# HiKapok/DAN

Hardware: AMD Instinct MI355X
Metric: 640x640 images/sec/node (train fwd+bwd) (higher is better)
Workload: dtype bf16; 1 GPU; S3FD VGG-16 backbone + 6 detection heads, 640x640 bf16 training (fwd+bwd+SGD), batch 16 per GPU; global_batch=16, parallelism=dp1, anchors_per_image=34125, step_launch=eager, rccl_ranks=1, weight_gradient_stream=True

## Files before the change

### dan_amd/_lib.py

```python
import ctypes
import os

import torch

_HERE = os.path.dirname(os.path.abspath(__file__))
ACT_NAME = os.environ.get("DANHIP_DTYPE", "bf16").lower()
if ACT_NAME not in ("bf16", "fp16"):
    raise ValueError("DANHIP_DTYPE must be bf16 or fp16, got %r" % ACT_NAME)
ACT_DTYPE = torch.float16 if ACT_NAME == "fp16" else torch.bfloat16
SO_PATH = os.path.join(_HERE, "libdanhip_f16.so" if ACT_NAME == "fp16" else "libdanhip.so")
if os.environ.get("DANHIP_LIB_PATH"):
    SO_PATH = os.path.abspath(os.environ["DANHIP_LIB_PATH"])

F32, BF16 = 0, 1
SPLIT3 = 3


class ConvDesc(ctypes.Structure):
    _fields_ = [(n, ctypes.c_int32) for n in ("N", "H", "W", "Cin", "Ho", "Wo", "Cout", "kh", "kw", "stride")]


class ConvPitch(ctypes.Structure):
    _fields_ = [(n, ctypes.c_int32) for n in ("x_pitch", "y_pitch", "aux_pitch")]

# ... 26 lines not shown
    "danhip_maxpool2x2_split3": [P, P, I32, I32, I32, I32, P],
    "danhip_l2norm_split3": [P, P, P, I64, I32, I32, I32, P],
    "danhip_conv3x3_c3_f32_split3": [P, P, P, P, I32, I32, I32, I32, ctypes.c_int, I32, P],
    "danhip_conv2d_fwd_split": [DESC, P, P, P, P, ctypes.c_int, ctypes.c_int, I32, P, ctypes.c_size_t, P],
    "danhip_l2norm_fwd_f32": [P, P, P, I64, I32, P],
    "danhip_resize_bilinear_add_fwd_f32": [P, P, P, I32, I32, I32, I32, I32, I32, P],
    "danhip_avgpool2x2s1_same_fwd_f32": [P, P, I32, I32, I32, I32, P],
    "danhip_deform_sample_fwd_f32": [P, P, P, I32, I32, I32, I32, I32, I32, I32, I32, I32, P],
    "danhip_conv2d_bwd_data": [DESC, P, P, P, P, ctypes.c_int, P],
    "danhip_conv2d_bwd_data_ws": [DESC, P, P, P, P, ctypes.c_int, P, ctypes.c_size_t, P],
    "danhip_conv2d_bwd_data_bits": [DESC, P, P, P, P, ctypes.c_int, P],
    "danhip_conv2d_bwd_data_bits_first": [DESC, P, P, P, P, I32, P, P, P],
    "danhip_relu_bits": [P, P, I64, I32, P],
    "danhip_conv2d_fwd_relu_bits": [DESC, P, P, P, P, P, P, P, P],
    "danhip_conv2d_bwd_weight": [DESC, P, P, P, P, I32, P],
    "danhip_conv2d_bwd_weight_ws": [DESC, P, P, P, P, I32, P, ctypes.c_size_t, P],
    "danhip_avgpool2x2s1_same_fwd_strided": [P, I32, P, I32, I32, I32, I32, I32, ctypes.c_int, P],
    "danhip_avgpool2x2s1_same_bwd_strided": [P, I32, P, I32, I32, I32, I32, I32, P],
    "danhip_add16": [P, P, P, I64, P],
    "danhip_residual_bwd": [P, P, P, P, P, ctypes.c_int, I64, P],
    "danhip_conv2d_fwd_strided": [DESC, P, P, P, P, ctypes.c_int, I32, ctypes.POINTER(ConvPitch), P, ctypes.c_size_t, P],
    "danhip_conv2d_bwd_data_strided": [DESC, P, P, P, P, ctypes.c_int, ctypes.POINTER(ConvPitch), P, ctypes.c_size_t, P],
    "danhip_conv2d_fwd_concat2": [DESC, P, P, I32, I32, P, P, P, ctypes.c_int, P],
    "danhip_conv2d_bwd_weight_strided": [DESC, P, P, P, P, I32, ctypes.POINTER(ConvPitch), P, ctypes.c_size_t, P],
    "danhip_relu_bwd_bias_grad": [P, P, P, I64, I32, P],
    "danhip_maxpool2x2_fwd": [P, P, I32, I32, I32, I32, P],
    "danhip_maxpool2x2_fwd_arg": [P, P, P, I32, I32, I32, I32, P],
    "danhip_maxpool2x2_bwd_arg": [P, P, P, I32, I32, I32, I32, ctypes.c_int, P],
    "danhip_conv2d_fwd_pool_arg": [DESC, P, P, P, P, P, P, P],
    "danhip_conv2d_fwd_relu_bits_arg": [DESC, P, P, P, P, P, P, P, P, P],
    "danhip_maxpool2x2_bwd": [P, P, P, I32, I32, I32, I32, ctypes.c_int, P],
    "danhip_l2norm_fwd": [P, P, P, I64, I32, P],
    "danhip_l2norm_bwd": [P, P, P, P, P, I64, I32, ctypes.c_int, ctypes.c_int, P],
    "danhip_preprocess_u8": [P, P, I64, P],
    "danhip_resize_bilinear_add_fwd": [P, P, P, I32, I32, I32, I32, I32, I32, P],
    "danhip_resize_bilinear_add_bwd": [P, P, I32, I32, I32, I32, I32, I32, ctypes.c_int, P],
    "danhip_avgpool2x2s1_same_fwd": [P, P, I32, I32, I32, I32, P],
    "danhip_avgpool2x2s1_same_bwd": [P, P, P, I32, I32, I32, I32, ctypes.c_int, P],
    "danhip_slice_deliver": [P, I32, I32, I32, P, I32, P, I32, ctypes.c_int, I64, P],
    "danhip_batchnorm_fwd_train": [P, P, P, P, P, P, P, P, I64, I32, FL, FL, ctypes.c_int, P, P],
    "danhip_batchnorm_fwd_infer": [P, P, P, P, P, P, I64, I32, ctypes.c_int, P],
    "danhip_batchnorm_bwd": [P, P, P, P, P, P, P, P, I64, I32, P],
    "danhip_dynamic_anchor_routing_eval": [P, P, P, P, I64, I32, I32, I32, I32, I32, P, P, P, ctypes.c_size_t, P],
    "danhip_dynamic_anchor_routing_train": [P, P, P, P, I64, I32, I32, I32, I32, I32, FL, FL, ctypes.c_uint64, ctypes.c_uint64, P, P, P, P,
                                            ctypes.c_size_t, P],
    "danhip_nms": [P, I32, I32, I32, FL, P, P, P],
    "danhip_argsort_desc_f32": [P, I64, I32, P, P, ctypes.c_size_t, P],
    "danhip_augment_preprocess": [P, I32, I32, I32, ctypes.POINTER(ctypes.c_int32), ctypes.POINTER(ctypes.c_float), I32, I32, I32, I32, I32, P, I32, I32,
                                  P, ctypes.c_size_t, P],
    "danhip_deform_psroi_pool_fwd": [P, P, P, P, P, I32, I32, I32, I32, I32, I32, I32, I32, I32, FL, FL, I32, I32, P],
    "danhip_deform_psroi_pool_bwd": [P, P, P, P, P, P, P, I32, I32, I32, I32, I32, I32, I32, I32, I32, I32, FL, FL, I32, I32, P],
    "danhip_maxpool3x3s2_same_fwd": [P, P, I32, I32, I32, I32, P],
    "danhip_maxpool3x3s2_same_bwd": [P, P, P, I32, I32, I32, I32, P],
    "danhip_resize_u8_linear": [P, I32, I32, P, I32, I32, I32, ctypes.c_double, ctypes.c_double, P],
    "danhip_bbox_vote": [P, P, I32, I32, ctypes.c_double, I32, P, P, P, ctypes.c_size_t, P],
    "danhip_deform_sample_fwd": [P, P, P, I32, I32, I32, I32, I32, I32, I32, I32, I32, P],
    "danhip_deform_sample_bwd": [P, P, P, P, P, I32, I32, I32, I32, I32, I32, I32, I32, I32, ctypes.c_int, P, ctypes.c_size_t, P],
    "danhip_deform_conv_fwd": [P, P, P, P, P, I32, I32, I32, I32, I32, I32, I32, I32, I32, I32, ctypes.c_int, P, ctypes.c_size_t, P],
    "danhip_deform_conv_bwd": [P, P, P, P, P, P, P, P, I32, I32, I32, I32, I32, I32, I32, I32, I32, I32, ctypes.c_int, P, ctypes.c_size_t, P],
    "danhip_deform_conv_bwd_with_col": [P, P, P, P, P, P, P, P, P, I32, I32, I32, I32, I32, I32, I32, I32, I32, I32, ctypes.c_int, P, ctypes.c_size_t, P],
    "danhip_deform_conv_bwd_deliver": [P, P, P, P, P, P, P, P, P, I32, I32, I32, I32, I32, I32, I32, I32, I32, I32, ctypes.c_int, ctypes.c_int, P, ctypes.c_size_t, P],
    "danhip_cast_pad_f32_to_bf16": [P, P, P, I64, I32, I32, P],
    "danhip_head_split_fwd": [P, P, P, I32, I32, I32, I32, I32, I32, I32, P],
    "danhip_head_split_bwd": [P, P, P, P, I32, I32, I32, I32, I32, I32, I32, P],
    "danhip_hard_neg_select": [P, P, P, P, P, P, I32, I32, FL, ctypes.c_int, P],
    "danhip_detection_loss_fwd": [P, P, P, P, P, P, P, P, I32, I32, P],
# ... 133 lines not shown
```

### dan_amd/csrc/elementwise.hip

```cpp
#include "common.h"

namespace {

__device__ __forceinline__ float wave_sum(float v) {
#pragma unroll
  for (int o = 32; o > 0; o >>= 1) v += __shfl_xor(v, o, 64);
  return v;
}

struct bf8 { uint4 v; };
__device__ __forceinline__ void unpack8(const uint4& u, float* f) {
  const unsigned w[4] = {u.x, u.y, u.z, u.w};
#pragma unroll
  for (int i = 0; i < 4; ++i) unpack2bf(w[i], f[2 * i], f[2 * i + 1]);
}
__device__ __forceinline__ uint4 pack8(const float* f) {
  uint4 u;
  u.x = pack2bf(f[0], f[1]); u.y = pack2bf(f[2], f[3]); u.z = pack2bf(f[4], f[5]); u.w = pack2bf(f[6], f[7]);
  return u;
}

__global__ void relu_bwd_bias_kernel(bf16_t* __restrict__ dy, const bf16_t* __restrict__ y, float* __restrict__ db, long M, int C) {
  const int cg = C / 8;
  const int tpr = blockDim.x / cg > 0 ? blockDim.x / cg : 1;
// ... 130 lines not shown
  const long nwaves = (long)gridDim.x * (blockDim.x >> 6);
  float gm[VPL][8];
#pragma unroll
  for (int v = 0; v < VPL; ++v)
#pragma unroll
    for (int i = 0; i < 8; ++i) gm[v][i] = gamma[(v * LPP + l) * 8 + i];
  for (long p0 = wave * PPW; p0 < M; p0 += nwaves * PPW) {
    const long pix = p0 + sub;
    const bool ok = pix < M;
    float f[VPL][8];
    float ss = 0.f;
#pragma unroll
    for (int v = 0; v < VPL; ++v) {
      if (ok) unpack8(*reinterpret_cast<const uint4*>(x + pix * C + (v * LPP + l) * 8), f[v]);
      else
#pragma unroll
        for (int i = 0; i < 8; ++i) f[v][i] = 0.f;
#pragma unroll
      for (int i = 0; i < 8; ++i) ss += f[v][i] * f[v][i];
    }
    ss = pixel_sum<LPP, VPL>(ss);
    const float inv = rsqrtf(fmaxf(ss, 1e-10f));
    if (ok) {
#pragma unroll
      for (int v = 0; v < VPL; ++v) {
#pragma unroll
        for (int i = 0; i < 8; ++i) f[v][i] = f[v][i] * inv * gm[v][i];
        *reinterpret_cast<uint4*>(y + pix * C + (v * LPP + l) * 8) = pack8(f[v]);
      }
    }
  }
}

template <int LPP, int VPL>
__global__ void l2norm_bwd_kernel(const bf16_t* __restrict__ x, const float* __restrict__ gamma, const bf16_t* __restrict__ dy,
                                  bf16_t* __restrict__ dx, float* __restrict__ dgamma, long M, int C, int accumulate, int relu_mask) {
  constexpr int PPW = 64 / LPP;
  extern __shared__ float sg[];
  for (int c = threadIdx.x; c < C; c += blockDim.x) sg[c] = 0.f;
  __syncthreads();
  const int lane = threadIdx.x & 63;
  const int sub = lane / LPP, l = lane % LPP;
  const long wave = (long)blockIdx.x * (blockDim.x >> 6) + (threadIdx.x >> 6);
  const long nwaves = (long)gridDim.x * (blockDim.x >> 6);
  float gm[VPL][8], dg[VPL][8];
#pragma unroll
  for (int v = 0; v < VPL; ++v)
#pragma unroll
    for (int i = 0; i < 8; ++i) { gm[v][i] = gamma[(v * LPP + l) * 8 + i]; dg[v][i] = 0.f; }
  for (long p0 = wave * PPW; p0 < M; p0 += nwaves * PPW) {
    const long pix = p0 + sub;
    const bool ok = pix < M;
    float f[VPL][8], g[VPL][8];
    float ss = 0.f, dot = 0.f;
#pragma unroll
    for (int v = 0; v < VPL; ++v) {
      const long o = pix * C + (v * LPP + l) * 8;
      if (ok) {
        unpack8(*reinterpret_cast<const uint4*>(x + o), f[v]);
        unpack8(*reinterpret_cast<const uint4*>(dy + o), g[v]);
      } else {
#pragma unroll
        for (int i = 0; i < 8; ++i) { f[v][i] = 0.f; g[v][i] = 0.f; }
      }
#pragma unroll
      for (int i = 0; i < 8; ++i) { ss += f[v][i] * f[v][i]; dot += g[v][i] * gm[v][i] * f[v][i]; }
    }
    ss = pixel_sum<LPP, VPL>(ss);
    dot = pixel_sum<LPP, VPL>(dot);
    const float inv = rsqrtf(fmaxf(ss, 1e-10f));
    const float k = (ss > 1e-10f) ? dot * inv * inv * inv : 0.f;
    if (ok) {
#pragma unroll
      for (int v = 0; v < VPL; ++v) {
        const long o = pix * C + (v * LPP + l) * 8;
        float r[8], old[8];
        if (accumulate) unpack8(*reinterpret_cast<const uint4*>(dx + o), old);
#pragma unroll
        for (int i = 0; i < 8; ++i) {
          float t = gm[v][i] * inv * g[v][i] - f[v][i] * k;
          if (relu_mask && !(f[v][i] > 0.f)) t = 0.f;
          if (accumulate) t += old[i];
          r[i] = t;
          dg[v][i] += g[v][i] * f[v][i] * inv;
        }
        *reinterpret_cast<uint4*>(dx + o) = pack8(r);
      }
    }
  }
#pragma unroll
  for (int v = 0; v < VPL; ++v)
#pragma unroll
    for (int i = 0; i < 8; ++i) atomicAdd(sg + (v * LPP + l) * 8 + i, dg[v][i]);
  __syncthreads();
  for (int c = threadIdx.x; c < C; c += blockDim.x) atomicAdd(dgamma + c, sg[c]);
}

__global__ void preprocess_kernel(const unsigned char* __restrict__ img, bf16_t* __restrict__ out, long npix) {
  for (long p = (long)blockIdx.x * blockDim.x + threadIdx.x; p < npix; p += (long)gridDim.x * blockDim.x) {
    const float r = (float)img[p * 3] - 123.68f, g = (float)img[p * 3 + 1] - 116.78f, b = (float)img[p * 3 + 2] - 103.94f;
    float f[8] = {b, g, r, 0, 0, 0, 0, 0};
    *reinterpret_cast<uint4*>(out + p * 8) = pack8(f);
  }
}

__global__ void cast_pad_kernel(const float* __restrict__ src, const bf16_t* __restrict__ relu_y, bf16_t* __restrict__ dst, long rows, int c_src,
                                int c_dst) {
  const long total = rows * c_dst;
  for (long i = (long)blockIdx.x * blockDim.x + threadIdx.x; i < total; i += (long)gridDim.x * blockDim.x) {
    const long r = i / c_dst;
    const int c = (int)(i % c_dst);
    float v = c < c_src ? src[r * c_src + c] : 0.f;
    if (relu_y && c < c_src && !(bf2f(relu_y[r * c_src + c]) > 0.f)) v = 0.f;
    dst[i] = f2bf(v);
  }
}

inline int grid_for(long total, int block, int cap = 8192) {
  long b = (total + block - 1) / block;
  if (b > cap) b = cap;
  if (b < 1) b = 1;
  return (int)b;
}

}

// ... 211 lines not shown
  const dim3 g((unsigned)blocks), b(256);
  switch (C) {
    case 64: hipLaunchKernelGGL((l2norm_fwd_kernel<8, 1>), g, b, 0, s, x, gamma, y, (long)M, C); break;
    case 128: hipLaunchKernelGGL((l2norm_fwd_kernel<16, 1>), g, b, 0, s, x, gamma, y, (long)M, C); break;
    case 256: hipLaunchKernelGGL((l2norm_fwd_kernel<32, 1>), g, b, 0, s, x, gamma, y, (long)M, C); break;
    case 512: hipLaunchKernelGGL((l2norm_fwd_kernel<64, 1>), g, b, 0, s, x, gamma, y, (long)M, C); break;
    default: hipLaunchKernelGGL((l2norm_fwd_kernel<64, 2>), g, b, 0, s, x, gamma, y, (long)M, C); break;
  }
  DH_LAUNCH_CHECK();
  return DANHIP_OK;
}

extern "C" int danhip_l2norm_bwd(const uint16_t* x, const float* gamma, const uint16_t* dy, uint16_t* dx, float* dgamma, int64_t M,
                                 int32_t C, int accumulate, int relu_mask, void* stream) {
  DH_REQUIRE(x && gamma && dy && dx && dgamma && M > 0, DANHIP_EINVAL, "l2norm_bwd: bad arguments");
  DH_REQUIRE(C == 256 || C == 512 || C == 1024 || C == 128 || C == 64, DANHIP_EINVAL, "l2norm_bwd: C=%d unsupported", C);
  hipStream_t s = (hipStream_t)stream;
  const int lpp = C >= 512 ? 64 : C / 8, ppw = 64 / lpp;
  long blocks = (M + 16 * ppw - 1) / (16 * ppw);
  if (blocks > 512) blocks = 512;
  const dim3 g((unsigned)blocks), b(1024);
  const size_t lds = (size_t)C * sizeof(float);
  switch (C) {
    case 64: hipLaunchKernelGGL((l2norm_bwd_kernel<8, 1>), g, b, lds, s, x, gamma, dy, dx, dgamma, (long)M, C, accumulate, relu_mask); break;
    case 128: hipLaunchKernelGGL((l2norm_bwd_kernel<16, 1>), g, b, lds, s, x, gamma, dy, dx, dgamma, (long)M, C, accumulate, relu_mask); break;
    case 256: hipLaunchKernelGGL((l2norm_bwd_kernel<32, 1>), g, b, lds, s, x, gamma, dy, dx, dgamma, (long)M, C, accumulate, relu_mask); break;
    case 512: hipLaunchKernelGGL((l2norm_bwd_kernel<64, 1>), g, b, lds, s, x, gamma, dy, dx, dgamma, (long)M, C, accumulate, relu_mask); break;
    default: hipLaunchKernelGGL((l2norm_bwd_kernel<64, 2>), g, b, lds, s, x, gamma, dy, dx, dgamma, (long)M, C, accumulate, relu_mask); break;
  }
  DH_LAUNCH_CHECK();
  return DANHIP_OK;
}

extern "C" int danhip_preprocess_u8(const uint8_t* img_rgb, uint16_t* out, int64_t npix, void* stream) {
  DH_REQUIRE(img_rgb && out && npix > 0, DANHIP_EINVAL, "preprocess_u8: bad arguments");
  hipLaunchKernelGGL(preprocess_kernel, dim3(grid_for(npix, 256)), dim3(256), 0, (hipStream_t)stream, img_rgb, out, (long)npix);
  DH_LAUNCH_CHECK();
  return DANHIP_OK;
}

extern "C" int danhip_cast_pad_f32_to_bf16(const float* src, const uint16_t* relu_y, uint16_t* dst, int64_t rows, int32_t c_src, int32_t c_dst,
                                           void* stream) {
  DH_REQUIRE(src && dst && rows > 0 && c_src > 0 && c_dst >= c_src, DANHIP_EINVAL, "cast_pad: bad arguments");
  hipLaunchKernelGGL(cast_pad_kernel, dim3(grid_for(rows * c_dst, 256)), dim3(256), 0, (hipStream_t)stream, src, relu_y, dst, (long)rows, c_src, c_dst);
  DH_LAUNCH_CHECK();
  return DANHIP_OK;
}
```

### dan_amd/ops.py

```python
import contextlib
import ctypes
import os

import torch

from . import _lib
from ._lib import ACT_DTYPE as ACT, BF16, F32, SPLIT3, ConvDesc, call, ptr, stream


class OpsContext(object):
    __slots__ = ("USE_SPLITK", "USE_SLOTS", "USE_RELU_BITS", "USE_POOL_ARG", "POOL_ONLY_TRAIN", "KEEP_DEFORM_COL", "WGRAD_STREAM", "WGRAD_FIRST", "FUSE_FIRST_WGRAD", "SPLIT_EVAL", "TRACE",
                 "PROFILE", "PROFILE_BYTES", "GRAD_READY_HOOK", "LOSS_SCALE_DEV", "wgrad")

    def __init__(self, **overrides):
        env = os.environ.get
        self.USE_SPLITK = True
        self.USE_SLOTS = True
        self.USE_RELU_BITS = env("DANHIP_RELU_BITS", "1") == "1"
        self.USE_POOL_ARG = env("DANHIP_POOL_ARG", "1") == "1"
        self.POOL_ONLY_TRAIN = env("DANHIP_POOL_ONLY_TRAIN", "1") == "1"
        self.KEEP_DEFORM_COL = True
        self.WGRAD_STREAM = env("DANHIP_WGRAD_STREAM", "1") == "1"
        self.WGRAD_FIRST = env("DANHIP_WGRAD_FIRST", "0") == "1"
        self.FUSE_FIRST_WGRAD = env("DANHIP_FUSE_FIRST_WGRAD", "1") == "1"
        self.SPLIT_EVAL = False
        self.TRACE = self.PROFILE = self.PROFILE_BYTES = None
        self.GRAD_READY_HOOK = self.LOSS_SCALE_DEV = None
        self.wgrad = {"on": False, "side": None, "main": None, "keep": []}
        for k, v in overrides.items():
            setattr(self, k, v)


_CTX = OpsContext()
_CTX_FIELDS = frozenset(OpsContext.__slots__) - {"wgrad"}


def context():
    return _CTX


@contextlib.contextmanager
def use_context(ctx):
    global _CTX
    prev, _CTX = _CTX, ctx
    try:
        yield ctx
    finally:
        _CTX = prev



def _desc(N, H, W, Cin, Cout, kh, kw, stride, valid=False):
# ... 136 lines not shown
        nbytes = 2.0 * d.N * (d.H * d.W * cin + out_px * co8) + 2.0 * d.kh * d.kw * cin * d.Cout
        _CTX.PROFILE_BYTES.setdefault(label, []).append(nbytes)




def wgrad_overlap_begin():
    if not torch.cuda.is_available():
        return
    if not _CTX.WGRAD_STREAM:
        return
    if _CTX.wgrad["side"] is None:
        _CTX.wgrad["side"] = torch.cuda.Stream()
    _CTX.wgrad["main"] = torch.cuda.current_stream()
    _CTX.wgrad["on"] = True


def wgrad_overlap_join():
    if _CTX.wgrad["on"]:
        torch.cuda.current_stream().wait_stream(_CTX.wgrad["side"])
    _CTX.wgrad["on"] = False
    _CTX.wgrad["keep"].clear()


def wgrad_streams():
    return [_CTX.wgrad["main"], _CTX.wgrad["side"]] if _CTX.wgrad["on"] else []





class GradSlot(object):

    __slots__ = ("shape", "dtype", "device", "is_relu", "buf", "count")

    def __init__(self, t, is_relu, channels=None):
        self.shape, self.dtype, self.device, self.is_relu = t.shape, t.dtype, t.device, is_relu
        if channels is not None:
            self.shape = tuple(t.shape[:-1]) + (channels,)
        self.buf, self.count = None, 0

    def target(self):
        if self.buf is None:
            self.buf = torch.empty(self.shape, dtype=self.dtype, device=self.device)
            self.count = 0
        acc = 1 if self.count > 0 else 0
        self.count += 1
        return self.buf, acc

    def take(self):
        b, n = self.buf, self.count
        self.buf, self.count = None, 0
        return b if n > 0 else None




def _slot_of(t):
    return getattr(t, "_dh_slot", None) if _CTX.USE_SLOTS else None


def _new_slot(track):
    return GradSlot.__new__(GradSlot) if (track and _CTX.USE_SLOTS) else None


def _attach_slot(t, is_relu):
    s = GradSlot(t, is_relu)
    t._dh_slot = s
    return s




def _bits_holder(x):
    h = getattr(x, "_dh_bits", None)
    if h is None:
        h = [None]
        x._dh_bits = h
    return h


def relu_bits(x, holder):
    if holder[0] is None:
        C = x.shape[-1]
        M = x.numel() // C
        b = torch.empty((M, C // 8), dtype=torch.uint8, device=x.device)
        call("danhip_relu_bits", ptr(x), ptr(b), M, C, stream())
        holder[0] = b
# ... 458 lines not shown
    if bits_out:
        y._dh_bits = [bits_out[0]]
    if yslot is not None:
        cout = w.shape[-1]
        if cout % 8 == 0:
            yslot.__init__(y, relu)
            y._dh_slot = yslot
        else:
            yslot.__init__(y, relu, (cout + 7) // 8 * 8)
            y._dh_pslot = yslot
    if pool_out:
        y._dh_pooled = pool_out[0]
        y._dh_pool_arg = pool_out[1]
        if bits_out and bits_out[1] is not None:
            y._dh_pooled_bits = bits_out[1]
    return y


class _MaxPool(torch.autograd.Function):

    @staticmethod
    def forward(ctx, x, xslot, yslot, pre=None, arg=None):
        N, H, W, C = x.shape
        if pre is not None:
            y = pre
        else:
            y = torch.empty((N, (H + 1) // 2, (W + 1) // 2, C), dtype=x.dtype, device=x.device)
            arg = _pool_arg_buffer(y, x.requires_grad and C % 8 == 0)
            call("danhip_maxpool2x2_fwd_arg", ptr(x), ptr(y), ptr(arg), N, H, W, C, stream())
        ctx.arg = arg
        ctx.save_for_backward(x if arg is None else None)
        ctx.dims = (N, H, W, C)
        ctx.xslot, ctx.yslot = xslot, yslot
        ctx.set_materialize_grads(False)
        return y

    @staticmethod
    def backward(ctx, dy):
        (x,) = ctx.saved_tensors
        N, H, W, C = ctx.dims
        g = ctx.yslot.take() if ctx.yslot is not None else None
        if dy is not None:
            g = dy.contiguous() if g is None else g.add_(dy)
        if g is None:
            return None, None, None, None, None

        def scatter(dst, acc):
            if ctx.arg is not None:
                call("danhip_maxpool2x2_bwd_arg", ptr(ctx.arg), ptr(g), ptr(dst), N, H, W, C, acc, stream())
            else:
                call("danhip_maxpool2x2_bwd", ptr(x), ptr(g), ptr(dst), N, H, W, C, acc, stream())

        if ctx.xslot is not None:
            buf, acc = ctx.xslot.target() if _pool_deliver_ok(ctx, dy) else (None, 0)
            if buf is not None:
                scatter(buf, acc)
                return None, None, None, None, None
        dx = torch.empty((N, H, W, C), dtype=g.dtype, device=g.device)
        scatter(dx, 0)
        return dx, None, None, None, None


def _pool_deliver_ok(ctx, dy):
    return not (ctx.xslot.is_relu and dy is not None)


def max_pool_2x2(x):
    if getattr(x, "_dh_already_pooled", False):
        return x
    if _is_limbs(x):
        N, H, W, C = x.shape
        if C % 8 == 0 and x._dh_split3.shape[-1] == 3 * C:
            y3 = torch.empty((N, (H + 1) // 2, (W + 1) // 2, 3 * C), dtype=torch.float16, device=x.device)
            call("danhip_maxpool2x2_split3", ptr(x._dh_split3), ptr(y3), N, H, W, C, stream())
            return _limb_view(y3, C, _limb_exp(x))
        x = unsplit3(x)
    if _f32_infer(x):
        N, H, W, C = x.shape
        y = torch.empty((N, (H + 1) // 2, (W + 1) // 2, C), dtype=torch.float32, device=x.device)
        call("danhip_maxpool2x2_fwd_f32", ptr(x.contiguous()), ptr(y), N, H, W, C, stream())
        return y
    if _CTX.TRACE is not None:
        _CTX.TRACE.setdefault("pools", []).append(x.detach())
    track = torch.is_grad_enabled() and x.requires_grad
    xs = _slot_of(x) if track else None
    yslot = _new_slot(track)
    y = _MaxPool.apply(x, xs, yslot, getattr(x, "_dh_pooled", None), getattr(x, "_dh_pool_arg", None))
    pbits = getattr(x, "_dh_pooled_bits", None)
    if pbits is not None and getattr(x, "_dh_pooled", None) is not None:
        y._dh_bits = [pbits]
    if yslot is not None:
        yslot.__init__(y, xs.is_relu if xs is not None else False)
        y._dh_slot = yslot
# ... 3 lines not shown
class _MaxPool3x3S2(torch.autograd.Function):

    @staticmethod
    def forward(ctx, x):
        N, H, W, C = x.shape
        y = torch.empty((N, (H + 1) // 2, (W + 1) // 2, C), dtype=x.dtype, device=x.device)
        call("danhip_maxpool3x3s2_same_fwd", ptr(x), ptr(y), N, H, W, C, stream())
        ctx.save_for_backward(x)
        return y

    @staticmethod
    def backward(ctx, dy):
        (x,) = ctx.saved_tensors
        N, H, W, C = x.shape
        dx = torch.empty_like(x)
        call("danhip_maxpool3x3s2_same_bwd", ptr(x), ptr(dy.contiguous()), ptr(dx), N, H, W, C, stream())
        return dx


def max_pool_3x3_s2(x):
    return _MaxPool3x3S2.apply(_f32_in(x))


class _L2Norm(torch.autograd.Function):

    @staticmethod
    def forward(ctx, x, gamma, g_param, xslot, yslot):
        y = torch.empty_like(x)
        M = x.numel() // x.shape[-1]
        call("danhip_l2norm_fwd", ptr(x), ptr(gamma.detach()), ptr(y), M, x.shape[-1], stream())
        ctx.save_for_backward(x, gamma.detach())
        ctx.g_param = g_param
        ctx.xslot, ctx.yslot = xslot, yslot
        ctx.set_materialize_grads(False)
        return y

    @staticmethod
    def backward(ctx, dy):
        x, gamma = ctx.saved_tensors
        M = x.numel() // x.shape[-1]
        g = ctx.yslot.take() if ctx.yslot is not None else None
        if dy is not None:
            g = dy.contiguous() if g is None else g.add_(dy)
        if g is None:
            return None, None, None, None, None
        sink = _grad_sink(ctx.g_param) if ctx.g_param is not None else None
        dg = sink if sink is not None else torch.zeros_like(gamma)
        xs = ctx.xslot
        if xs is not None:
            buf, acc = xs.target()
            call("danhip_l2norm_bwd", ptr(x), ptr(gamma), ptr(g), ptr(buf), ptr(dg), M, x.shape[-1], acc, 1 if xs.is_relu else 0, stream())
            dx = None
        else:
            dx = torch.empty_like(x)
            call("danhip_l2norm_bwd", ptr(x), ptr(gamma), ptr(g), ptr(dx), ptr(dg), M, x.shape[-1], 0, 0, stream())
        return dx, (None if sink is not None else dg), None, None, None


def l2_normalize(x, gamma):
    if _is_limbs(x) and x.shape[-1] % 8 == 0 and x._dh_split3.shape[-1] == 3 * x.shape[-1]:
        C = x.shape[-1]
        y3 = torch.empty_like(x._dh_split3)
        _range_flag(x.device)
        call("danhip_l2norm_split3", ptr(x._dh_split3), ptr(gamma.detach().float()), ptr(y3), y3.numel() // (3 * C), C, _limb_exp(x), 0, stream())
        return _limb_view(y3, C)
    x = _f32_in(x)
    if _f32_infer(x):
        y = torch.empty_like(x)
        call("danhip_l2norm_fwd_f32", ptr(x.contiguous()), ptr(gamma.detach()), ptr(y), x.numel() // x.shape[-1], x.shape[-1], stream())
        return y
    track = torch.is_grad_enabled() and (x.requires_grad or gamma.requires_grad)
    yslot = _new_slot(track)
    y = _L2Norm.apply(x, gamma, gamma if isinstance(gamma, torch.nn.Parameter) else None, _slot_of(x) if track else None, yslot)
    if yslot is not None:
        yslot.__init__(y, False)
        y._dh_slot = yslot
    return y


class _HeadSplit(torch.autograd.Function):

    @staticmethod
    def forward(ctx, h, loc, cls, nneg, npos, off):
        B, H, W, Ch = h.shape
# ... 802 lines not shown
```

### include/danhip.h

```cpp
#ifndef DANHIP_H_
#define DANHIP_H_
#include <stddef.h>
#include <stdint.h>

#ifdef __cplusplus
extern "C" {
#endif

#define DANHIP_OK 0
#define DANHIP_EINVAL (-1)
#define DANHIP_ELAUNCH (-2)
#define DANHIP_EWORKSPACE (-3)

#define DANHIP_F32 0
#define DANHIP_BF16 1
#define DANHIP_F16 2
#define DANHIP_SPLIT3 3

const char* danhip_last_error(void);
int danhip_version(void);
int danhip_set_option(const char* name, int value);
int danhip_get_option(const char* name);
int danhip_act_dtype(void);

// ... 49 lines not shown

int danhip_conv2d_fwd_concat2_supported(const danhip_conv_desc* d, int32_t c1, int32_t src_pitch);
int danhip_conv2d_fwd_concat2(const danhip_conv_desc* d, const uint16_t* x1, const uint16_t* x2, int32_t c1, int32_t src_pitch,
                              const uint16_t* wf_packed, const float* bias, uint16_t* y, int relu, void* stream);

typedef struct { int32_t x_pitch, y_pitch, aux_pitch; } danhip_conv_pitch;
int danhip_conv2d_fwd_strided(const danhip_conv_desc* d, const uint16_t* x, const uint16_t* wf_packed, const float* bias, uint16_t* y,
                              int relu, int32_t relu_channels, const danhip_conv_pitch* pitch, void* ws, size_t ws_bytes, void* stream);
int danhip_conv2d_bwd_data_strided(const danhip_conv_desc* d, const uint16_t* dy, const uint16_t* wb_packed, const uint16_t* relu_mask,
                                   uint16_t* dx, int accumulate, const danhip_conv_pitch* pitch, void* ws, size_t ws_bytes, void* stream);
int danhip_conv2d_bwd_weight_strided(const danhip_conv_desc* d, const uint16_t* x, const uint16_t* dy, float* dw_hwio, float* db,
                                     int32_t cin_real, const danhip_conv_pitch* pitch, void* ws, size_t ws_bytes, void* stream);

int danhip_conv2d_bwd_weight(const danhip_conv_desc* d, const uint16_t* x, const uint16_t* dy, float* dw_hwio, float* db,
                             int32_t cin_real, void* stream);
size_t danhip_conv2d_bwd_weight_workspace_bytes(const danhip_conv_desc* d);
int danhip_conv2d_bwd_weight_ws(const danhip_conv_desc* d, const uint16_t* x, const uint16_t* dy, float* dw_hwio, float* db,
                                int32_t cin_real, void* ws, size_t ws_bytes, void* stream);

int danhip_relu_bwd_bias_grad(uint16_t* dy, const uint16_t* y, float* db, int64_t M, int32_t C, void* stream);

const char* danhip_conv_kernel_label(const danhip_conv_desc* d, int which);
const char* danhip_conv_wgrad_kernel_label(const danhip_conv_desc* d);

int danhip_maxpool2x2_fwd(const uint16_t* x, uint16_t* y, int32_t N, int32_t H, int32_t W, int32_t C, void* stream);
int danhip_maxpool2x2_bwd(const uint16_t* x, const uint16_t* dy, uint16_t* dx, int32_t N, int32_t H, int32_t W, int32_t C,
                          int accumulate, void* stream);
int danhip_maxpool2x2_fwd_arg(const uint16_t* x, uint16_t* y, uint8_t* arg, int32_t N, int32_t H, int32_t W, int32_t C, void* stream);
int danhip_maxpool2x2_bwd_arg(const uint8_t* arg, const uint16_t* dy, uint16_t* dx, int32_t N, int32_t H, int32_t W, int32_t C,
                              int accumulate, void* stream);
int danhip_l2norm_fwd(const uint16_t* x, const float* gamma, uint16_t* y, int64_t M, int32_t C, void* stream);
int danhip_l2norm_bwd(const uint16_t* x, const float* gamma, const uint16_t* dy, uint16_t* dx, float* dgamma, int64_t M,
                      int32_t C, int accumulate, int relu_mask, void* stream);
int danhip_resize_bilinear_add_fwd(const uint16_t* up, const uint16_t* lateral, uint16_t* out, int32_t N, int32_t Hi, int32_t Wi,
                                   int32_t Ho, int32_t Wo, int32_t C, void* stream);
int danhip_resize_bilinear_add_bwd(const uint16_t* dout, uint16_t* dup, int32_t N, int32_t Hi, int32_t Wi, int32_t Ho, int32_t Wo,
                                   int32_t C, int accumulate, void* stream);
int danhip_avgpool2x2s1_same_fwd(const uint16_t* x, uint16_t* y, int32_t N, int32_t H, int32_t W, int32_t C, void* stream);
int danhip_avgpool2x2s1_same_bwd(const uint16_t* dy, const uint16_t* x_mask, uint16_t* dx, int32_t N, int32_t H, int32_t W, int32_t C,
                                 int accumulate, void* stream);
int danhip_add16(const uint16_t* a, const uint16_t* b, uint16_t* out, int64_t n, void* stream);
int danhip_residual_bwd(const uint16_t* dy, const uint16_t* r, const uint16_t* x_mask, uint16_t* dr, uint16_t* dx, int accumulate, int64_t n,
                        void* stream);
int danhip_avgpool2x2s1_same_fwd_strided(const uint16_t* x, int32_t x_pitch, uint16_t* y, int32_t y_pitch, int32_t N, int32_t H, int32_t W,
                                         int32_t C, int relu, void* stream);
int danhip_avgpool2x2s1_same_bwd_strided(const uint16_t* dy, int32_t y_pitch, uint16_t* dx, int32_t x_pitch, int32_t N, int32_t H, int32_t W,
                                         int32_t C, void* stream);
int danhip_slice_deliver(const uint16_t* dy, int32_t ldy, int32_t c0, int32_t C, const uint16_t* mask, int32_t ldm, uint16_t* out, int32_t Cpad,
                         int accumulate, int64_t M, void* stream);
int danhip_batchnorm_fwd_train(const uint16_t* x, const float* gamma, const float* beta, uint16_t* y, float* save_mean,
                               float* save_rstd, float* moving_mean, float* moving_var, int64_t M, int32_t C, float eps,
                               float momentum, int relu, float* workspace, void* stream);
int danhip_batchnorm_fwd_infer(const uint16_t* x, const float* gamma, const float* beta, const float* mean, const float* rstd,
                               uint16_t* y, int64_t M, int32_t C, int relu, void* stream);
int danhip_batchnorm_bwd(const uint16_t* x, const uint16_t* dy, const float* gamma, const float* save_mean, const float* save_rstd,
                         uint16_t* dx, float* dgamma, float* dbeta, int64_t M, int32_t C, void* stream);
int danhip_preprocess_u8(const uint8_t* img_rgb, uint16_t* out, int64_t npix, void* stream);
int danhip_cast_pad_f32_to_bf16(const float* src, const uint16_t* relu_y, uint16_t* dst, int64_t rows, int32_t c_src, int32_t c_dst,
                                void* stream);

int danhip_head_split_fwd(const float* h, float* loc, float* cls, int32_t B, int32_t HW, int32_t Ch, int32_t nneg, int32_t npos,
                          int32_t A, int32_t anchor_offset, void* stream);
int danhip_head_split_bwd(const float* h, const float* dloc, const float* dcls, float* dy, int32_t B, int32_t HW, int32_t Ch,
                          int32_t nneg, int32_t npos, int32_t A, int32_t anchor_offset, void* stream);
int danhip_hard_neg_select(const float* cls, const int32_t* labels, float* score, int32_t* counts, float* thr, int32_t* k_out,
                           int32_t B, int32_t A, float negative_ratio, int at_least_one, void* stream);
// ... 149 lines not shown
```

Measured before the change: 1307 images/sec.

## Fuse L2Norm backward with maxpool-backward scatter at shared junction tensors

Adds a kernel that computes the L2Norm backward and the 2x2 maxpool argmax scatter for the same input tensor in one pass, writing the summed gradient once. A deferred-delivery mechanism in GradSlot holds the first contribution until the second arrives, then dispatches the fused kernel. This removes a separate read-modify-write of the full-resolution gradient buffer at the conv3_3/conv4_3/conv5_3 taps. It rounds in the same order as the two-kernel path to keep numerics matching, and adds deferred-state bookkeeping that could misfire if delivery order differs.

```diff
diff --git a/dan_amd/_lib.py b/dan_amd/_lib.py
--- a/dan_amd/_lib.py
+++ b/dan_amd/_lib.py
@@ -82,6 +82,7 @@
     "danhip_maxpool2x2_bwd": [P, P, P, I32, I32, I32, I32, ctypes.c_int, P],
     "danhip_l2norm_fwd": [P, P, P, I64, I32, P],
     "danhip_l2norm_bwd": [P, P, P, P, P, I64, I32, ctypes.c_int, ctypes.c_int, P],
+    "danhip_l2norm_bwd_pool_scatter": [P, P, P, P, P, P, P, I32, I32, I32, I32, ctypes.c_int, ctypes.c_int, ctypes.c_int, P],
     "danhip_preprocess_u8": [P, P, I64, P],
     "danhip_resize_bilinear_add_fwd": [P, P, P, I32, I32, I32, I32, I32, I32, P],
     "danhip_resize_bilinear_add_bwd": [P, P, I32, I32, I32, I32, I32, I32, ctypes.c_int, P],
diff --git a/dan_amd/csrc/elementwise.hip b/dan_amd/csrc/elementwise.hip
--- a/dan_amd/csrc/elementwise.hip
+++ b/dan_amd/csrc/elementwise.hip
@@ -186,6 +186,22 @@
   }
 }
 
+__device__ __forceinline__ void l2_bwd_sums(const float* f, const float* g, const float* gm, float& ss, float& dot) {
+#pragma clang fp contract(off)
+#pragma unroll
+  for (int i = 0; i < 8; ++i) { ss = ss + f[i] * f[i]; dot = __builtin_fmaf(g[i] * gm[i], f[i], dot); }
+}
+__device__ __forceinline__ float l2_bwd_term(float f, float g, float gm, float inv, float k, int relu_mask) {
+#pragma clang fp contract(off)
+  float t = gm * inv * g - f * k;
+  if (relu_mask && !(f > 0.f)) t = 0.f;
+  return t;
+}
+__device__ __forceinline__ float l2_bwd_dgamma(float dg, float f, float g, float inv) {
+#pragma clang fp contract(off)
+  return __builtin_fmaf(g * f, inv, dg);
+}
+
 template <int LPP, int VPL>
 __global__ void l2norm_bwd_kernel(const bf16_t* __restrict__ x, const float* __restrict__ gamma, const bf16_t* __restrict__ dy,
                                   bf16_t* __restrict__ dx, float* __restrict__ dgamma, long M, int C, int accumulate, int relu_mask) {
@@ -217,8 +233,7 @@
 #pragma unroll
         for (int i = 0; i < 8; ++i) { f[v][i] = 0.f; g[v][i] = 0.f; }
       }
-#pragma unroll
-      for (int i = 0; i < 8; ++i) { ss += f[v][i] * f[v][i]; dot += g[v][i] * gm[v][i] * f[v][i]; }
+      l2_bwd_sums(f[v], g[v], gm[v], ss, dot);
     }
     ss = pixel_sum<LPP, VPL>(ss);
     dot = pixel_sum<LPP, VPL>(dot);
@@ -232,11 +247,10 @@
         if (accumulate) unpack8(*reinterpret_cast<const uint4*>(dx + o), old);
 #pragma unroll
         for (int i = 0; i < 8; ++i) {
-          float t = gm[v][i] * inv * g[v][i] - f[v][i] * k;
-          if (relu_mask && !(f[v][i] > 0.f)) t = 0.f;
+          float t = l2_bwd_term(f[v][i], g[v][i], gm[v][i], inv, k, relu_mask);
           if (accumulate) t += old[i];
           r[i] = t;
-          dg[v][i] += g[v][i] * f[v][i] * inv;
+          dg[v][i] = l2_bwd_dgamma(dg[v][i], f[v][i], g[v][i], inv);
         }
         *reinterpret_cast<uint4*>(dx + o) = pack8(r);
       }
@@ -246,6 +260,91 @@
   for (int v = 0; v < VPL; ++v)
 #pragma unroll
     for (int i = 0; i < 8; ++i) atomicAdd(sg + (v * LPP + l) * 8 + i, dg[v][i]);
+  __syncthreads();
+  for (int c = threadIdx.x; c < C; c += blockDim.x) atomicAdd(dgamma + c, sg[c]);
+}
+
+template <int LPP>
+__global__ __launch_bounds__(512) void l2norm_bwd_pool_scatter_kernel(const bf16_t* __restrict__ x, const float* __restrict__ gamma,
+                                                                      const bf16_t* __restrict__ dy, const unsigned char* __restrict__ arg,
+                                                                      const bf16_t* __restrict__ pdy, bf16_t* __restrict__ dx,
+                                                                      float* __restrict__ dgamma, int N, int H, int W, int C, int Ho, int Wo,
+                                                                      int accumulate, int relu_mask, int pool_first) {
+  constexpr int PPW = 64 / LPP;
+  extern __shared__ float sg[];
+  for (int c = threadIdx.x; c < C; c += blockDim.x) sg[c] = 0.f;
+  __syncthreads();
+  const int lane = threadIdx.x & 63;
+  const int sub = lane / LPP, l = lane % LPP;
+  const long wave = (long)blockIdx.x * (blockDim.x >> 6) + (threadIdx.x >> 6);
+  const long nwaves = (long)gridDim.x * (blockDim.x >> 6);
+  const long NW = (long)N * Ho * Wo;
+  float gm[8], dg[8];
+#pragma unroll
+  for (int i = 0; i < 8; ++i) { gm[i] = gamma[l * 8 + i]; dg[i] = 0.f; }
+  const uint4 z = make_uint4(0, 0, 0, 0);
+  for (long w0 = wave * PPW; w0 < NW; w0 += nwaves * PPW) {
+    const long win = w0 + sub;
+    const bool okw = win < NW;
+    long p = okw ? win : 0;
+    const int wo = (int)(p % Wo); p /= Wo;
+    const int ho = (int)(p % Ho);
+    const int n = (int)(p / Ho);
+    unsigned codes = 0;
+    uint4 gyr = z, xr[4], gr[4];
+    long off[4];
+    bool ok[4];
+#pragma unroll
+    for (int t = 0; t < 4; ++t) {
+      const int h = ho * 2 + (t >> 1), w = wo * 2 + (t & 1);
+      ok[t] = okw && h < H && w < W;
+      off[t] = (((long)n * H + h) * W + w) * C + l * 8;
+      xr[t] = ok[t] ? *reinterpret_cast<const uint4*>(x + off[t]) : z;
+      gr[t] = ok[t] ? *reinterpret_cast<const uint4*>(dy + off[t]) : z;
+    }
+    if (okw) {
+      codes = *reinterpret_cast<const unsigned short*>(arg + win * (C / 4) + l * 2);
+      gyr = *reinterpret_cast<const uint4*>(pdy + win * C + l * 8);
+    }
+    float gy[8];
+    unpack8(gyr, gy);
+#pragma unroll
+    for (int t = 0; t < 4; ++t) {
+      float f[8], g[8];
+      unpack8(xr[t], f);
+      unpack8(gr[t], g);
+      float ss = 0.f, dot = 0.f;
+      l2_bwd_sums(f, g, gm, ss, dot);
+      ss = pixel_sum<LPP, 1>(ss);
+      dot = pixel_sum<LPP, 1>(dot);
+      const float inv = rsqrtf(fmaxf(ss, 1e-10f));
+      const float k = (ss > 1e-10f) ? dot * inv * inv * inv : 0.f;
+      if (ok[t]) {
+        float a[8], b[8], old[8];
+        if (accumulate) unpack8(*reinterpret_cast<const uint4*>(dx + off[t]), old);
+#pragma unroll
+        for (int i = 0; i < 8; ++i) {
+          b[i] = l2_bwd_term(f[i], g[i], gm[i], inv, k, relu_mask);
+          a[i] = (((codes >> (2 * i)) & 3u) == (unsigned)t) ? gy[i] : 0.f;
+          dg[i] = l2_bwd_dgamma(dg[i], f[i], g[i], inv);
+        }
+        if (!pool_first) {
+#pragma unroll
+          for (int i = 0; i < 8; ++i) { const float s = a[i]; a[i] = b[i]; b[i] = s; }
+        }
+        if (accumulate) {
+#pragma unroll
+          for (int i = 0; i < 8; ++i) a[i] += old[i];
+        }
+        unpack8(pack8(a), a);
+#pragma unroll
+        for (int i = 0; i < 8; ++i) b[i] += a[i];
+        *reinterpret_cast<uint4*>(dx + off[t]) = pack8(b);
+      }
+    }
+  }
+#pragma unroll
+  for (int i = 0; i < 8; ++i) atomicAdd(sg + l * 8 + i, dg[i]);
   __syncthreads();
   for (int c = threadIdx.x; c < C; c += blockDim.x) atomicAdd(dgamma + c, sg[c]);
 }
@@ -523,6 +622,36 @@
   return DANHIP_OK;
 }
 
+extern "C" int danhip_l2norm_bwd_pool_scatter(const uint16_t* x, const float* gamma, const uint16_t* dy, const uint8_t* arg, const uint16_t* pooled_dy,
+                                              uint16_t* dx, float* dgamma, int32_t N, int32_t H, int32_t W, int32_t C, int accumulate,
+                                              int relu_mask, int pool_first, void* stream) {
+  DH_REQUIRE(x && gamma && dy && arg && pooled_dy && dx && dgamma && N > 0 && H > 0 && W > 0, DANHIP_EINVAL, "l2norm_bwd_pool_scatter: bad arguments");
+  DH_REQUIRE(C == 64 || C == 128 || C == 256 || C == 512, DANHIP_EINVAL, "l2norm_bwd_pool_scatter: C=%d unsupported", C);
+  hipStream_t s = (hipStream_t)stream;
+  const int Ho = (H + 1) / 2, Wo = (W + 1) / 2;
+  const int lpp = C / 8, ppw = 64 / lpp;
+  const long nwin = (long)N * Ho * Wo;
+  long blocks = (nwin + 8 * ppw - 1) / (8 * ppw);
+  if (blocks > 512) {
+    const long sweeps = (blocks + 511) / 512;
+    blocks = (blocks + sweeps - 1) / sweeps;
+  }
+  const dim3 g((unsigned)blocks), b(512);
+  const size_t lds = (size_t)C * sizeof(float);
+#define DH_JUNCTION(LPP) \
+  hipLaunchKernelGGL((l2norm_bwd_pool_scatter_kernel<LPP>), g, b, lds, s, x, gamma, dy, arg, pooled_dy, dx, dgamma, N, H, W, C, Ho, Wo, accumulate, \
+                     relu_mask, pool_first)
+  switch (C) {
+    case 64: DH_JUNCTION(8); break;
+    case 128: DH_JUNCTION(16); break;
+    case 256: DH_JUNCTION(32); break;
+    default: DH_JUNCTION(64); break;
+  }
+#undef DH_JUNCTION
+  DH_LAUNCH_CHECK();
+  return DANHIP_OK;
+}
+
 extern "C" int danhip_preprocess_u8(const uint8_t* img_rgb, uint16_t* out, int64_t npix, void* stream) {
   DH_REQUIRE(img_rgb && out && npix > 0, DANHIP_EINVAL, "preprocess_u8: bad arguments");
   hipLaunchKernelGGL(preprocess_kernel, dim3(grid_for(npix, 256)), dim3(256), 0, (hipStream_t)stream, img_rgb, out, (long)npix);
diff --git a/dan_amd/ops.py b/dan_amd/ops.py
--- a/dan_amd/ops.py
+++ b/dan_amd/ops.py
@@ -9,7 +9,7 @@
 
 
 class OpsContext(object):
-    __slots__ = ("USE_SPLITK", "USE_SLOTS", "USE_RELU_BITS", "USE_POOL_ARG", "POOL_ONLY_TRAIN", "KEEP_DEFORM_COL", "WGRAD_STREAM", "WGRAD_FIRST", "FUSE_FIRST_WGRAD", "SPLIT_EVAL", "TRACE",
+    __slots__ = ("USE_SPLITK", "USE_SLOTS", "USE_RELU_BITS", "USE_POOL_ARG", "USE_JUNCTION", "POOL_ONLY_TRAIN", "KEEP_DEFORM_COL", "WGRAD_STREAM", "WGRAD_FIRST", "FUSE_FIRST_WGRAD", "SPLIT_EVAL", "TRACE",
                  "PROFILE", "PROFILE_BYTES", "GRAD_READY_HOOK", "LOSS_SCALE_DEV", "wgrad")
 
     def __init__(self, **overrides):
@@ -18,6 +18,7 @@
         self.USE_SLOTS = True
         self.USE_RELU_BITS = env("DANHIP_RELU_BITS", "1") == "1"
         self.USE_POOL_ARG = env("DANHIP_POOL_ARG", "1") == "1"
+        self.USE_JUNCTION = env("DANHIP_JUNCTION", "1") == "1"
         self.POOL_ONLY_TRAIN = env("DANHIP_POOL_ONLY_TRAIN", "1") == "1"
         self.KEEP_DEFORM_COL = True
         self.WGRAD_STREAM = env("DANHIP_WGRAD_STREAM", "1") == "1"
@@ -220,15 +221,33 @@
 
 class GradSlot(object):
 
-    __slots__ = ("shape", "dtype", "device", "is_relu", "buf", "count")
+    __slots__ = ("shape", "dtype", "device", "is_relu", "buf", "count", "taps", "pending")
 
     def __init__(self, t, is_relu, channels=None):
         self.shape, self.dtype, self.device, self.is_relu = t.shape, t.dtype, t.device, is_relu
         if channels is not None:
             self.shape = tuple(t.shape[:-1]) + (channels,)
         self.buf, self.count = None, 0
+        self.taps, self.pending = 0, None
+
+    def defer(self, kind, alone, payload):
+        buf, acc = self.target()
+        self.pending = (kind, acc, alone, payload)
+
+    def pop_pending(self, kind):
+        p = self.pending
+        if p is None or p[0] != kind:
+            return None
+        self.pending = None
+        return p[1], p[3]
+
+    def flush(self):
+        p, self.pending = self.pending, None
+        if p is not None:
+            p[2](self.buf, p[1])
 
     def target(self):
+        self.flush()
         if self.buf is None:
             self.buf = torch.empty(self.shape, dtype=self.dtype, device=self.device)
             self.count = 0
@@ -237,11 +256,19 @@
         return self.buf, acc
 
     def take(self):
+        self.flush()
         b, n = self.buf, self.count
         self.buf, self.count = None, 0
         return b if n > 0 else None
 
 
+
+
+TAP_L2NORM, TAP_POOL = 1, 2
+
+
+def _junction_ok(slot, dy, C):
+    return _CTX.USE_JUNCTION and slot.taps == (TAP_L2NORM | TAP_POOL) and dy is None and C in (64, 128, 256, 512)
 
 
 def _slot_of(t):
@@ -766,6 +793,8 @@
         ctx.save_for_backward(x if arg is None else None)
         ctx.dims = (N, H, W, C)
         ctx.xslot, ctx.yslot = xslot, yslot
+        if xslot is not None and arg is not None:
+            xslot.taps |= TAP_POOL
         ctx.set_materialize_grads(False)
         return y
 
@@ -786,13 +815,31 @@
                 call("danhip_maxpool2x2_bwd", ptr(x), ptr(g), ptr(dst), N, H, W, C, acc, stream())
 
         if ctx.xslot is not None:
-            buf, acc = ctx.xslot.target() if _pool_deliver_ok(ctx, dy) else (None, 0)
+            xs = ctx.xslot
+            if ctx.arg is not None and _pool_deliver_ok(ctx, dy) and _junction_ok(xs, dy, C):
+                first = xs.pop_pending(TAP_L2NORM)
+                if first is not None:
+                    buf, _ = xs.target()
+                    _junction(first[1], (ctx.arg, g, (N, H, W, C)), buf, first[0], xs.is_relu, 0)
+                elif xs.pending is None:
+                    xs.defer(TAP_POOL, scatter, (ctx.arg, g, (N, H, W, C)))
+                else:
+                    scatter(*xs.target())
+                return None, None, None, None, None
+            buf, acc = xs.target() if _pool_deliver_ok(ctx, dy) else (None, 0)
             if buf is not None:
                 scatter(buf, acc)
                 return None, None, None, None, None
         dx = torch.empty((N, H, W, C), dtype=g.dtype, device=g.device)
         scatter(dx, 0)
         return dx, None, None, None, None
+
+
+def _junction(l2, pool, buf, acc, is_relu, pool_first):
+    x, gamma, g, dg = l2
+    arg, pg, (N, H, W, C) = pool
+    call("danhip_l2norm_bwd_pool_scatter", ptr(x), ptr(gamma), ptr(g), ptr(arg), ptr(pg), ptr(buf), ptr(dg), N, H, W, C, acc, 1 if is_relu else 0,
+         pool_first, stream())
 
 
 def _pool_deliver_ok(ctx, dy):
@@ -862,6 +909,8 @@
         ctx.save_for_backward(x, gamma.detach())
         ctx.g_param = g_param
         ctx.xslot, ctx.yslot = xslot, yslot
+        if xslot is not None and x.dim() == 4:
+            xslot.taps |= TAP_L2NORM
         ctx.set_materialize_grads(False)
         return y
 
@@ -878,8 +927,17 @@
         dg = sink if sink is not None else torch.zeros_like(gamma)
         xs = ctx.xslot
         if xs is not None:
-            buf, acc = xs.target()
-            call("danhip_l2norm_bwd", ptr(x), ptr(gamma), ptr(g), ptr(buf), ptr(dg), M, x.shape[-1], acc, 1 if xs.is_relu else 0, stream())
+            def alone(buf, acc):
+                call("danhip_l2norm_bwd", ptr(x), ptr(gamma), ptr(g), ptr(buf), ptr(dg), M, x.shape[-1], acc, 1 if xs.is_relu else 0, stream())
+
+            first = xs.pop_pending(TAP_POOL) if _junction_ok(xs, dy, x.shape[-1]) else None
+            if first is not None:
+                buf, _ = xs.target()
+                _junction((x, gamma, g, dg), first[1], buf, first[0], xs.is_relu, 1)
+            elif sink is not None and _junction_ok(xs, dy, x.shape[-1]) and xs.pending is None:
+                xs.defer(TAP_L2NORM, alone, (x, gamma, g, dg))
+            else:
+                alone(*xs.target())
             dx = None
         else:
             dx = torch.empty_like(x)
diff --git a/include/danhip.h b/include/danhip.h
--- a/include/danhip.h
+++ b/include/danhip.h
@@ -105,6 +105,9 @@
 int danhip_l2norm_fwd(const uint16_t* x, const float* gamma, uint16_t* y, int64_t M, int32_t C, void* stream);
 int danhip_l2norm_bwd(const uint16_t* x, const float* gamma, const uint16_t* dy, uint16_t* dx, float* dgamma, int64_t M,
                       int32_t C, int accumulate, int relu_mask, void* stream);
+int danhip_l2norm_bwd_pool_scatter(const uint16_t* x, const float* gamma, const uint16_t* dy, const uint8_t* arg, const uint16_t* pooled_dy,
+                                   uint16_t* dx, float* dgamma, int32_t N, int32_t H, int32_t W, int32_t C, int accumulate, int relu_mask,
+                                   int pool_first, void* stream);
 int danhip_resize_bilinear_add_fwd(const uint16_t* up, const uint16_t* lateral, uint16_t* out, int32_t N, int32_t Hi, int32_t Wi,
                                    int32_t Ho, int32_t Wo, int32_t C, void* stream);
 int danhip_resize_bilinear_add_bwd(const uint16_t* dout, uint16_t* dup, int32_t N, int32_t Hi, int32_t Wi, int32_t Ho, int32_t Wo,
```

After: 1329 images/sec (median of 6 runs). 1.02x the previous value.
